# liruiw/OMG-Planner

Hardware: AMD Instinct MI355X
Metric: CHOMP iterations/sec (batched scenes) + ms/plan, Panda 7-DoF 30-wp (higher is better)
Workload: dtype f32 SDF / f64 kinematics+update; 1 GPU; 100 table-top scenes/GPU x (64-goal goal-set cost + CHOMP step), Panda 9-dof, 30 waypoints; scenes_per_gpu=100, total_scenes=100, goals=64, waypoints=30, sdf_grid=4x64^3 + 128x96x32 per scene, private, goal_selection=MD on device (omgx_goal_update_optimize), pipeline_parts=3, top_k_collision=1000, plan_restart_every_steps=50

## Files before the change

### omg-planner_amd/csrc/omg_device.h

```cpp
#pragma once
#include <hip/hip_runtime.h>
#include <stdint.h>

#include "../../include/omg_hip.h"

#define OMG_WAVE 64

namespace omg {

struct __attribute__((packed, aligned(4))) F2 { float a, b; };
struct __attribute__((packed, aligned(4))) F4 { float a, b, c, d; };

__device__ __forceinline__ float lerpf(float a, float b, float t) { return __builtin_fmaf(t, b - a, a); }

struct Axis { int i0; float f; bool ok; };
__device__ __forceinline__ Axis axis_of(float g) {
    Axis a;
    a.ok = (g > -1.0e9f) && (g <= 1.0e9f);
    const float s = g - 0.5f;
    a.i0 = (int)s;
    a.f = s - (float)a.i0;
    const bool edge = (s == -1.0f) && (g > -0.5f);
    a.i0 = edge ? 0 : a.i0;
    a.f = edge ? -1.0f : a.f;
// ... 165 lines not shown
        fmx = sdf_value(G, axm, ay, az);
        fmy = sdf_value(G, ax, aym, az);
        fmz = sdf_value(G, ax, ay, azm);
    }
    const float g0 = (float)(0.5 * (double)(fpx - fmx) * o.rdelta);
    const float g1 = (float)(0.5 * (double)(fpy - fmy) * o.rdelta);
    const float g2 = (float)(0.5 * (double)(fpz - fmz) * o.rdelta);
    float v0, v1, v2;
    if (value <= 0.0f) {
        acc.pot += (float)(-(double)value + 0.5 * (double)o.eps);
        v0 = -g0; v1 = -g1; v2 = -g2;
    } else {
        const float d = value - o.eps;
        acc.pot += o.i2eps * d * d * o.pad;
        const float ie = o.ieps;
        v0 = ie * g0 * d * o.pad; v1 = ie * g1 * d * o.pad; v2 = ie * g2 * d * o.pad;
    }
    acc.gx += __builtin_fmaf(T[8], v2, __builtin_fmaf(T[4], v1, T[0] * v0));
    acc.gy += __builtin_fmaf(T[9], v2, __builtin_fmaf(T[5], v1, T[1] * v0));
    acc.gz += __builtin_fmaf(T[10], v2, __builtin_fmaf(T[6], v1, T[2] * v0));
}

template <bool WANT_GRAD>
__device__ __forceinline__ void sdf_pair(const ObjParams& o, const float* __restrict__ grid, float px, float py, float pz,
                                         Accum& acc) {
    const PairPrep pp = pair_prepare(o, px, py, pz);
    if (!pp.far) pair_exact<WANT_GRAD>(o, grid, pp.tx, pp.ty, pp.tz, acc);
}

#define OMG_CONST_AS __attribute__((address_space(4)))
typedef const OMG_CONST_AS omgx_object* ObjTablePtr;
typedef const OMG_CONST_AS int32_t* IntTablePtr;
#define OMG_GLOBAL_AS __attribute__((address_space(1)))
typedef const OMG_GLOBAL_AS char* GlobalBytes;
typedef float F2v __attribute__((ext_vector_type(2), aligned(4)));
__device__ __forceinline__ F2 global_f2(GlobalBytes p) { const F2v v = *(const OMG_GLOBAL_AS F2v*)p; return F2{v.x, v.y}; }
__device__ __forceinline__ ObjTablePtr as_const(const omgx_object* p) { return (ObjTablePtr)(uintptr_t)p; }
__device__ __forceinline__ IntTablePtr as_const(const int32_t* p) { return (IntTablePtr)(uintptr_t)p; }

__device__ __forceinline__ ObjParams load_object(ObjTablePtr ob) {
    ObjParams o;
#pragma unroll
    for (int k = 0; k < 12; ++k) o.T[k] = ob->pose_inv[k];
#pragma unroll
    for (int k = 0; k < 3; ++k) { o.lo[k] = ob->lo[k]; o.hi[k] = ob->hi[k]; o.dim[k] = ob->dim[k]; }
    o.delta = ob->delta; o.eps = ob->epsilon; o.pad = ob->padding_scale; o.clr = ob->clearance;
#pragma unroll
    for (int k = 0; k < 3; ++k) { o.rw[k] = ob->inv_extent[k]; o.rc[k] = ob->rb_c[k]; o.rh[k] = ob->rb_h[k]; }
    o.rr2 = ob->rb_r2;
    o.rdelta = ob->inv_delta; o.i2eps = ob->inv_2eps; o.ieps = ob->inv_eps;
    return o;
}

template <bool WANT_GRAD>
__device__ __forceinline__ Accum sdf_point(const omgx_object* __restrict__ objs, int o_begin, int o_end,
                                           const float* __restrict__ pool, float px, float py, float pz) {
    Accum acc{0.0f, 0.0f, 0.0f, 0.0f, 0.0f};
    for (int o = o_begin; o < o_end; ++o) {
        ObjTablePtr ob = as_const(objs) + o;
        if (ob->disabled > 0) continue;
        const ObjParams op = load_object(ob);
        sdf_pair<WANT_GRAD>(op, pool + ob->grid_offset, px, py, pz, acc);
    }
    return acc;
}

__device__ __forceinline__ void gq_warm_scalar_cache(const omgx_object* objects, int o_begin, int o_end, const double* balls) {
    const omgx_object* ob[8];
#pragma unroll
    for (int k = 0; k < 8; ++k) ob[k] = objects + (o_begin + k < o_end ? o_begin + k : o_end - 1);
#define OMG_WARM_OBJ(N) "s_load_dword s96, %" #N ", 0x0\n\ts_load_dword s97, %" #N ", 0x40\n\ts_load_dword s98, %" #N ", 0x80\n\ts_load_dword s99, %" #N ", 0xb4\n\t"
    asm volatile(OMG_WARM_OBJ(0) OMG_WARM_OBJ(1) OMG_WARM_OBJ(2) OMG_WARM_OBJ(3) OMG_WARM_OBJ(4) OMG_WARM_OBJ(5) OMG_WARM_OBJ(6) OMG_WARM_OBJ(7)
                 "s_load_dword s96, %8, 0x0\n\ts_load_dword s97, %8, 0x40\n\ts_load_dword s98, %8, 0x80\n\ts_load_dword s99, %8, 0xc0\n\t"
                 "s_load_dword s96, %8, 0x100\n\ts_load_dword s97, %8, 0x13c\n\ts_waitcnt lgkmcnt(0)"
                 :
                 : "s"(ob[0]), "s"(ob[1]), "s"(ob[2]), "s"(ob[3]), "s"(ob[4]), "s"(ob[5]), "s"(ob[6]), "s"(ob[7]), "s"(balls)
                 : "s96", "s97", "s98", "s99", "memory");
#undef OMG_WARM_OBJ
}

template <class DPtr>
struct RobotViewT {
    const double* __restrict__ raw;
    DPtr d;
    const double* __restrict__ g;
    int P;
    __device__ __forceinline__ RobotViewT(const double* blob, int P_) : raw(blob), d((DPtr)(uintptr_t)(blob + OMGX_ROBOT_POINTS + 30 * P_)), g(blob + OMGX_ROBOT_POINTS + 30 * P_), P(P_) {}
    __device__ __forceinline__ RobotViewT(const double* blob, int P_, DPtr chain_constants) : raw(blob), d(chain_constants), g(blob + OMGX_ROBOT_POINTS + 30 * P_), P(P_) {}
    __device__ __forceinline__ DPtr uvw(int i) const { return d + 27 * i; }
    __device__ __forceinline__ DPtr tp(int i) const { return d + 189 + 3 * i; }
    __device__ __forceinline__ DPtr hand() const { return d + 210; }
    __device__ __forceinline__ DPtr lf() const { return d + 222; }
    __device__ __forceinline__ DPtr rf() const { return d + 234; }
    __device__ __forceinline__ const double* pts(int l, int p) const { return g + 246 + 3 * (l * P + p); }
    __device__ __forceinline__ DPtr ax(int l) const { return d + 246 + 30 * P + 3 * l; }
    __device__ __forceinline__ DPtr og(int l) const { return d + 276 + 30 * P + 3 * l; }
    __device__ __forceinline__ double radius(int l) const { return d[306 + 30 * P + l]; }
    __device__ __forceinline__ DPtr ball(int l) const { return d + 316 + 30 * P + 4 * l; }
    __device__ __forceinline__ const double* lower() const { return raw + OMGX_ROBOT_LOWER; }
    __device__ __forceinline__ const double* upper() const { return raw + OMGX_ROBOT_UPPER; }
};
typedef RobotViewT<const double*> RobotView;
typedef RobotViewT<const OMG_CONST_AS double*> RobotViewS;

struct Pose { double R[9]; double t[3]; };

// ... 42 lines not shown
            nxt.t[r] = cur.R[3 * r] * tp[0] + cur.R[3 * r + 1] * tp[1] + cur.R[3 * r + 2] * tp[2] + cur.t[r];
        }
        cur = nxt;
        f(i, cur);
    }
    Pose hand;
    pose_mul(cur, rv.hand(), hand);
    f(7, hand);
    {
        double Fm[12];
        const auto L = rv.lf();
#pragma unroll
        for (int k = 0; k < 12; ++k) Fm[k] = L[k];
        Fm[7] += deg_round_trip(q[7]);
        Pose fp;
        pose_mul(hand, Fm, fp);
        f(8, fp);
        const auto Rr = rv.rf();
#pragma unroll
        for (int k = 0; k < 12; ++k) Fm[k] = Rr[k];
        Fm[7] -= deg_round_trip(q[8]);
        pose_mul(hand, Fm, fp);
        f(9, fp);
    }
}

__device__ __forceinline__ void fk_joint_sincos(double q, double& s, double& c) { sincos(deg_round_trip(q), &s, &c); }

__device__ __forceinline__ double fk_dot3(double a0, double a1, double a2, double b0, double b1, double b2) {
#pragma clang fp contract(off)
    return __builtin_fma(a2, b2, __builtin_fma(a1, b1, a0 * b0));
}
__device__ __forceinline__ double fk_bentry(double c, double s, double U, double V, double W) {
#pragma clang fp contract(off)
    return __builtin_fma(s, V, c * U) + W;
}
template <class RV, class F>
__device__ __forceinline__ void fk_chain_tail(const RV& rv, double a0, double a1, double a2, double at, double q7, double q8, F&& f) {
#pragma clang fp contract(off)
    const auto H = rv.hand();
    const double h0 = fk_dot3(a0, a1, a2, H[0], H[4], H[8]), h1 = fk_dot3(a0, a1, a2, H[1], H[5], H[9]), h2 = fk_dot3(a0, a1, a2, H[2], H[6], H[10]);
    const double ht = fk_dot3(a0, a1, a2, H[3], H[7], H[11]) + at;
    f(7, h0, h1, h2, ht);
    const auto Lf = rv.lf();
    f(8, fk_dot3(h0, h1, h2, Lf[0], Lf[4], Lf[8]), fk_dot3(h0, h1, h2, Lf[1], Lf[5], Lf[9]), fk_dot3(h0, h1, h2, Lf[2], Lf[6], Lf[10]),
      fk_dot3(h0, h1, h2, Lf[3], Lf[7] + deg_round_trip(q7), Lf[11]) + ht);
    const auto Rf = rv.rf();
    f(9, fk_dot3(h0, h1, h2, Rf[0], Rf[4], Rf[8]), fk_dot3(h0, h1, h2, Rf[1], Rf[5], Rf[9]), fk_dot3(h0, h1, h2, Rf[2], Rf[6], Rf[10]),
      fk_dot3(h0, h1, h2, Rf[3], Rf[7] - deg_round_trip(q8), Rf[11]) + ht);
}

template <class RV, class F>
__device__ __forceinline__ void fk_chain_row(const RV& rv, int r, const double* __restrict__ sc ,
                                             double q7, double q8, F&& f) {
#pragma clang fp contract(off)
    double a0 = r == 0 ? 1.0 : 0.0, a1 = r == 1 ? 1.0 : 0.0, a2 = r == 2 ? 1.0 : 0.0, at = 0.0;
#pragma unroll 1
    for (int i = 0; i < 7; ++i) {
        const double s = sc[2 * i], c = sc[2 * i + 1];
        const auto uvw = rv.uvw(i);
        const auto tp = rv.tp(i);
        double B[9];
#pragma unroll
        for (int k = 0; k < 9; ++k) B[k] = fk_bentry(c, s, uvw[k], uvw[9 + k], uvw[18 + k]);
        const double n0 = fk_dot3(a0, a1, a2, B[0], B[3], B[6]);
        const double n1 = fk_dot3(a0, a1, a2, B[1], B[4], B[7]);
        const double n2 = fk_dot3(a0, a1, a2, B[2], B[5], B[8]);
        at = fk_dot3(a0, a1, a2, tp[0], tp[1], tp[2]) + at;
        a0 = n0; a1 = n1; a2 = n2;
        f(i, a0, a1, a2, at);
    }
    fk_chain_tail(rv, a0, a1, a2, at, q7, q8, f);
}

template <class RV>
__device__ __forceinline__ void fk_joint_matrix(const RV& rv, int i, double s, double c, double* __restrict__ B) {
    const auto uvw = rv.uvw(i);
#pragma unroll
    for (int k = 0; k < 9; ++k) B[k] = fk_bentry(c, s, uvw[k], uvw[9 + k], uvw[18 + k]);
}

template <class RV, class F>
__device__ __forceinline__ void fk_chain_row_B(const RV& rv, int r, const double* Bt , double q7, double q8, F&& f, int bstride = 9) {
#pragma clang fp contract(off)
    double a0 = r == 0 ? 1.0 : 0.0, a1 = r == 1 ? 1.0 : 0.0, a2 = r == 2 ? 1.0 : 0.0, at = 0.0;
#pragma unroll 1
    for (int i = 0; i < 7; ++i) {
        const double* B = Bt + bstride * i;
        const auto tp = rv.tp(i);
        const double n0 = fk_dot3(a0, a1, a2, B[0], B[3], B[6]);
        const double n1 = fk_dot3(a0, a1, a2, B[1], B[4], B[7]);
        const double n2 = fk_dot3(a0, a1, a2, B[2], B[5], B[8]);
        at = fk_dot3(a0, a1, a2, tp[0], tp[1], tp[2]) + at;
        a0 = n0; a1 = n1; a2 = n2;
        f(i, a0, a1, a2, at);
    }
    fk_chain_tail(rv, a0, a1, a2, at, q7, q8, f);
}

__device__ __forceinline__ void pose_apply(const Pose& A, const double* __restrict__ p, double& x, double& y, double& z) {
#pragma clang fp contract(fast)
    x = A.R[0] * p[0] + A.R[1] * p[1] + A.R[2] * p[2] + A.t[0];
    y = A.R[3] * p[0] + A.R[4] * p[1] + A.R[5] * p[2] + A.t[1];
    z = A.R[6] * p[0] + A.R[7] * p[1] + A.R[8] * p[2] + A.t[2];
}

__device__ __forceinline__ void pose12_apply(const double* __restrict__ A, const double* __restrict__ p, float& x, float& y, float& z) {
#pragma clang fp contract(fast)
    x = (float)(A[0] * p[0] + A[1] * p[1] + A[2] * p[2] + A[9]);
    y = (float)(A[3] * p[0] + A[4] * p[1] + A[5] * p[2] + A[10]);
    z = (float)(A[6] * p[0] + A[7] * p[1] + A[8] * p[2] + A[11]);
}

__device__ __forceinline__ void pose9_apply(const double* __restrict__ A, const double* __restrict__ p, float& x, float& y, float& z) {
#pragma clang fp contract(fast)
    const double r20 = A[1] * A[5] - A[2] * A[4], r21 = A[2] * A[3] - A[0] * A[5], r22 = A[0] * A[4] - A[1] * A[3];
    x = (float)(A[0] * p[0] + A[1] * p[1] + A[2] * p[2] + A[6]);
    y = (float)(A[3] * p[0] + A[4] * p[1] + A[5] * p[2] + A[7]);
    z = (float)(r20 * p[0] + r21 * p[1] + r22 * p[2] + A[8]);
}

template <class BP>
__device__ __forceinline__ void link_ball_center(const double* r0, const double* r1, const double* t, BP b, float& cx, float& cy, float& cz) {
#pragma clang fp contract(off)
    const double c0 = b[0], c1 = b[1], c2 = b[2];
    const double r20 = __builtin_fma(r0[1], r1[2], -(r0[2] * r1[1])), r21 = __builtin_fma(r0[2], r1[0], -(r0[0] * r1[2])),
                 r22 = __builtin_fma(r0[0], r1[1], -(r0[1] * r1[0]));
    cx = (float)(fk_dot3(r0[0], r0[1], r0[2], c0, c1, c2) + t[0]);
    cy = (float)(fk_dot3(r1[0], r1[1], r1[2], c0, c1, c2) + t[1]);
    cz = (float)(fk_dot3(r20, r21, r22, c0, c1, c2) + t[2]);
}

template <bool MIN>
__device__ __forceinline__ bool np_arg_better(double v, int i, double bv, int bi) {
    const bool vn = v != v, bn = bv != bv;
    if (vn | bn) return vn && (!bn || i < bi);
    return (MIN ? v < bv : v > bv) || (v == bv && i < bi);
}

template <int CTRL>
__device__ __forceinline__ int dpp_i32(int v) { return __builtin_amdgcn_update_dpp(0, v, CTRL, 0xf, 0xf, false); }
template <int CTRL>
__device__ __forceinline__ float dpp_f32(float v) { return __int_as_float(dpp_i32<CTRL>(__float_as_int(v))); }
template <int CTRL>
__device__ __forceinline__ double dpp_f64(double v) {
    return __hiloint2double(dpp_i32<CTRL>(__double2hiint(v)), dpp_i32<CTRL>(__double2loint(v)));
}
__device__ __forceinline__ int wave_suffix_sum_i32(int v) {
    v += __builtin_amdgcn_update_dpp(0, v, 0x101, 0xf, 0xf, true);
    v += __builtin_amdgcn_update_dpp(0, v, 0x102, 0xf, 0xf, true);
// ... 37 lines not shown
```

### omg-planner_amd/csrc/omg_goalset_queue.h

```cpp
#pragma once

#define GQ_TBL_MAX 32
#ifndef GQ_WG_PER_CU
#define GQ_WG_PER_CU 5
#endif
#ifndef GQ_WAVES
#define GQ_WAVES 4
#endif
#define GQ_NT (64 * GQ_WAVES)

struct GqFar {
    float T[12], lo[3], rc[3], rh[3], rr2, rb_r;
    bool cullable;
    int disabled;
};

typedef uint32_t GqU16 __attribute__((ext_vector_type(16)));
typedef uint32_t GqU8 __attribute__((ext_vector_type(8)));
typedef uint32_t GqU4 __attribute__((ext_vector_type(4)));
static_assert(offsetof(omgx_object, pose_inv) == 0 && offsetof(omgx_object, lo) == 0x30 && offsetof(omgx_object, epsilon) == 0x58 &&
              offsetof(omgx_object, clearance) == 0x60 && offsetof(omgx_object, disabled) == 0x64 && offsetof(omgx_object, rb_c) == 0x88 &&
              offsetof(omgx_object, rb_h) == 0x94 && offsetof(omgx_object, rb_r) == 0xa0 && offsetof(omgx_object, rb_r2) == 0xa4 &&
              sizeof(omgx_object) >= 0xa8, "gq_load_far reads the record by byte offsets");
__device__ __forceinline__ GqFar gq_load_far(ObjTablePtr ob) {
    GqU16 a;
    GqU4 b;
    GqU8 c;
    asm volatile("s_load_dwordx16 %0, %3, 0x0\n\ts_load_dwordx4 %1, %3, 0x58\n\ts_load_dwordx8 %2, %3, 0x88\n\ts_waitcnt lgkmcnt(0)"
                 : "=&s"(a), "=&s"(b), "=&s"(c) : "s"((uint64_t)(uintptr_t)ob));
    GqFar f;
#pragma unroll
    for (int k = 0; k < 12; ++k) f.T[k] = __uint_as_float(a[k]);
#pragma unroll
    for (int k = 0; k < 3; ++k) { f.lo[k] = __uint_as_float(a[12 + k]); f.rc[k] = __uint_as_float(c[k]); f.rh[k] = __uint_as_float(c[3 + k]); }
    f.rb_r = __uint_as_float(c[6]);
    f.rr2 = __uint_as_float(c[7]);
    f.cullable = ((int32_t)b[0] < 0x3f800000) & ((int32_t)b[2] <= 0x3f800000);
    f.disabled = (int32_t)b[3];
    return f;
}
__device__ __forceinline__ void se3_apply_s(const float* T, float x, float y, float z, float& ux, float& uy, float& uz) {
    ux = T[3]; uy = T[7]; uz = T[11];
    asm("v_fma_f32 %0, %3, %12, %0\n\tv_fma_f32 %1, %6, %12, %1\n\tv_fma_f32 %2, %9, %12, %2\n\t"
        "v_fma_f32 %0, %4, %13, %0\n\tv_fma_f32 %1, %7, %13, %1\n\tv_fma_f32 %2, %10, %13, %2\n\t"
        "v_fma_f32 %0, %5, %14, %0\n\tv_fma_f32 %1, %8, %14, %1\n\tv_fma_f32 %2, %11, %14, %2"
        : "+v"(ux), "+v"(uy), "+v"(uz)
        : "s"(T[0]), "s"(T[1]), "s"(T[2]), "s"(T[4]), "s"(T[5]), "s"(T[6]), "s"(T[8]), "s"(T[9]), "s"(T[10]), "v"(x), "v"(y), "v"(z));
}
__device__ __forceinline__ unsigned long long wave_ballot(bool b) { return __builtin_amdgcn_ballot_w64(b); }

struct GqLayout {
    int mask_off, tile_off, tbl_off, pts_off, stage_off, fkc_off, objc_off, btab_off, total;
    __host__ __device__ GqLayout(int PS, int MR, int P, int tbl_n, bool with_fkc = false, int waves = GQ_WAVES) {
        mask_off = PS * 90 * 8;
        tile_off = mask_off + 10 * MR * 4;
        tbl_off = mask_off + ((10 * MR * 4 + 16 + 15) & ~15);
        pts_off = tbl_off + tbl_n * 64;
        stage_off = pts_off + ((10 * P * 3 * 8 + 15) & ~15);
        total = stage_off + waves * 64 * 16;
        const int fk = stage_off + PS * 14 * 8 + 16;
        if (total < fk) total = fk;
        total = (total + 15) & ~15;
        fkc_off = total;
        if (with_fkc) total += 246 * 8;
        objc_off = total;
        if (with_fkc) total += 8 * 64 * 5 * 4;
        btab_off = total;
        if (with_fkc) total += PS * 7 * 9 * 8;
    }
};

static inline int gq_choose_tbl_n(int PS, int MR, int P, bool with_fkc = false, int waves = GQ_WAVES) {
    static const int step[] = {26624, 31744, 40960, 53248, 80896, 163840};
    const int base = GqLayout(PS, MR, P, 0, with_fkc, waves).total;
    for (int k = 0; k < 6; ++k)
        if (base + 4 * 64 <= step[k]) {
            const int n = (step[k] - base) / 64;
            return n < GQ_TBL_MAX ? n : GQ_TBL_MAX;
        }
    return 0;
}

struct GqTblRec { double rw[3]; int32_t dim[3]; int64_t goffb; float eps, clr, pad, i2e; };
__device__ __forceinline__ GqTblRec gq_tbl_load(const omgx_object* ob) {
    GqTblRec r;
#pragma unroll
    for (int k = 0; k < 3; ++k) { r.rw[k] = ob->inv_extent[k]; r.dim[k] = ob->dim[k]; }
    r.goffb = ob->grid_offset * 4;
    r.eps = ob->epsilon; r.clr = ob->clearance; r.pad = ob->padding_scale; r.i2e = ob->inv_2eps;
    return r;
}
__device__ __forceinline__ void gq_tbl_store(uint32_t* e, const GqTblRec& r) {
#pragma unroll
// ... 690 lines not shown
```

### omg-planner_amd/csrc/omg_kernels.hip

```cpp
#include <hip/hip_runtime.h>
#include <hip/hip_ext.h>

#include <stdint.h>
#include <stdio.h>
#include <stdlib.h>
#include <string.h>

#include <mutex>

#include "omg_device.h"
#include "omg_host.h"

using namespace omg;

struct RawObjects {
    const float* __restrict__ pose_init;
    const float* __restrict__ sdf_grids;
    const float* __restrict__ sdf_limits;
    const float* __restrict__ eps;
    const float* __restrict__ pad;
    const float* __restrict__ clr;
    const float* __restrict__ dis;
};

// ... 239 lines not shown
                        if (!__any((many & bit) != 0)) continue;
                        ObjTablePtr ob = as_const(a.objects) + o;
                        if (ob->disabled > 0) continue;
                        const ObjParams op = load_object(ob);
                        const float* grid = a.pool + ob->grid_offset;
                        PairPrep pp[LB];
#pragma unroll
                        for (int k = 0; k < LB; ++k) {
                            pp[k] = pair_prepare(op, px[k], py[k], pz[k]);
                            pp[k].far = pp[k].far || !(msk[k] & bit);
                        }
#pragma unroll
                        for (int k = 0; k < LB; ++k)
                            if (!pp[k].far) pair_exact<WANT_GRAD>(op, grid, pp[k].tx, pp[k].ty, pp[k].tz, acc[k]);
                    }
                }
#pragma unroll
                for (int k = 0; k < LB; ++k) {
                    const int l = l0 + k;
                    if (a.soften && l >= 8) {
                        acc[k].pot *= 0.1f; acc[k].gx *= 0.1f; acc[k].gy *= 0.1f; acc[k].gz *= 0.1f; acc[k].col = 0.0f;
                    }
                    if (a.arc && acc[k].pot != 0.0f) {
                        float qx, qy, qz;
                        pose12_apply(ci > 0 ? base + ((int64_t)l * pstride + ci - 1) * 12 : sbase + (int64_t)l * sstride, rv.pts(l, p), qx, qy, qz);
                        const float vx = (px[k] - qx) * a.inv_dt, vy = (py[k] - qy) * a.inv_dt, vz = (pz[k] - qz) * a.inv_dt;
                        acc[k].pot = acc[k].pot * sqrtf(vx * vx + vy * vy + vz * vz);
                    }
                    const int64_t kk = (out_cfg + l) * P + p;
                    if (a.pot) a.pot[kk] = acc[k].pot;
                    if (a.col) a.col[kk] = acc[k].col;
                    if (WANT_GRAD) { a.grad[3 * kk] = acc[k].gx; a.grad[3 * kk + 1] = acc[k].gy; a.grad[3 * kk + 2] = acc[k].gz; }
                    tsum += acc[k].pot;
                    tcol += acc[k].col;
                }
            }
        }
    }
    if (a.chunk_cost || a.chunk_col) {
        const float ws_ = wave_sum(tsum), wc_ = wave_sum(tcol);
        const int w = threadIdx.x >> 6;
        if ((threadIdx.x & 63) == 0) { red[0][w] = ws_; red[1][w] = wc_; }
        __syncthreads();
        if (threadIdx.x == 0) {
            const int64_t k = (int64_t)s * a.NCH + chunk;
            float c0 = red[0][0], c1 = red[1][0];
#pragma unroll
            for (int w2 = 1; w2 < TPB / 64; ++w2) { c0 += red[0][w2]; c1 += red[1][w2]; }
            if (a.chunk_cost) a.chunk_cost[k] = c0;
            if (a.chunk_col) a.chunk_col[k] = c1;
        }
    }
}
template <bool LAT, bool PERSIST = false>
__device__ __forceinline__ void waypoint_layer_block(const ChunkArgs& a, const int s, const int l_begin, const int l_end,
                                                     const int c_begin, const int c_end, double* lds_pose, uint32_t* rowmask,
                                                     const int o_begin, const int o_end, const RobotViewS& rv, double* fkc,
                                                     const bool warming, float* objc, double* btab) {
    const int n = a.wp_n, P = a.P, PS = a.PS, MR = a.MR;
    const int nloc = c_end - c_begin;
    const double* tr = a.wp_traj + ((int64_t)s * n + c_begin) * 9;
    double* sc = reinterpret_cast<double*>(rowmask);
    auto ldtr = [&](int k) -> double {
        if constexpr (PERSIST) return __hip_atomic_load(tr + k, __ATOMIC_RELAXED, __HIP_MEMORY_SCOPE_AGENT);
        else return tr[k];
    };
    const double fkv = (LAT && threadIdx.x < 246) ? rv.g[threadIdx.x] : 0.0;
    if (warming) gq_warm_scalar_cache(a.objects, o_begin, o_end, a.robot + OMGX_ROBOT_POINTS + 30 * P + 316 + 30 * P);
    for (int t = threadIdx.x; t < nloc * 7; t += 256) {
        const int cfg = t / 7, i = t - cfg * 7;
        double sn, cs;
        fk_joint_sincos(ldtr(cfg * 9 + i), sn, cs);
        sc[2 * t] = sn; sc[2 * t + 1] = cs;
    }
    if (LAT && threadIdx.x < 246) fkc[threadIdx.x] = fkv;
    __syncthreads();
    double* const gpose = (a.wp_pose_out && l_begin == 0) ? a.wp_pose_out + ((int64_t)s * n + c_begin) * 120 : nullptr;
    auto run_chain = [&](const auto& view) {
        for (int t = threadIdx.x; t < nloc * 3; t += 256) {
            const int cfg = t / 3, r = t - cfg * 3;
            fk_chain_row(view, r, sc + 14 * cfg, ldtr(cfg * 9 + 7), ldtr(cfg * 9 + 8), [&](int l, double r0, double r1, double r2, double tt) {
                double* dst = lds_pose + ((size_t)l * PS + cfg) * 9;
                if (r < 2) { dst[3 * r] = r0; dst[3 * r + 1] = r1; dst[3 * r + 2] = r2; }
                dst[6 + r] = tt;
                if (gpose) {
                    double* g = gpose + ((size_t)cfg * 10 + l) * 12;
                    g[3 * r] = r0; g[3 * r + 1] = r1; g[3 * r + 2] = r2; g[9 + r] = tt;
                }
            });
        }
    };
    if constexpr (LAT) {
        const RobotView rvl(a.robot, P, fkc);
        for (int t = threadIdx.x; t < nloc * 7; t += 256) fk_joint_matrix(rvl, t - (t / 7) * 7, sc[2 * t], sc[2 * t + 1], btab + 9 * t);
        __syncthreads();
        for (int t = threadIdx.x; t < nloc * 3; t += 256) {
            const int cfg = t / 3, r = t - cfg * 3;
            fk_chain_row_B(rvl, r, btab + 63 * cfg, ldtr(cfg * 9 + 7), ldtr(cfg * 9 + 8), [&](int l, double r0, double r1, double r2, double tt) {
                double* dst = lds_pose + ((size_t)l * PS + cfg) * 9;
                if (r < 2) { dst[3 * r] = r0; dst[3 * r + 1] = r1; dst[3 * r + 2] = r2; }
                dst[6 + r] = tt;
                if (gpose) {
                    double* g = gpose + ((size_t)cfg * 10 + l) * 12;
                    g[3 * r] = r0; g[3 * r + 1] = r1; g[3 * r + 2] = r2; g[9 + r] = tt;
                }
            });
        }
    } else run_chain(rv);
    __syncthreads();
    for (int row = l_begin * nloc + threadIdx.x; row < l_end * nloc; row += 256) {
        const int l = row / nloc, ci = row - l * nloc;
        const double* A = lds_pose + ((int64_t)l * PS + ci) * 9;
        const auto bl = rv.ball(l);
        float cx, cy, cz;
        link_ball_center(A, A + 3, A + 6, bl, cx, cy, cz);
        const float rad = (float)bl[3] + 1.0e-4f;
        uint32_t m = 0;
        for (int o = o_begin; o < o_end; ++o) {
            ObjTablePtr ob = as_const(a.objects) + o;
            if (ob->disabled > 0) continue;
            const int oo = o - o_begin;
            const uint32_t bit = 1u << (oo < 31 ? oo : 31);
            const float ux = __builtin_fmaf(ob->pose_inv[2], cz, __builtin_fmaf(ob->pose_inv[1], cy, __builtin_fmaf(ob->pose_inv[0], cx, ob->pose_inv[3]))) - ob->lo[0];
            const float uy = __builtin_fmaf(ob->pose_inv[6], cz, __builtin_fmaf(ob->pose_inv[5], cy, __builtin_fmaf(ob->pose_inv[4], cx, ob->pose_inv[7]))) - ob->lo[1];
            const float uz = __builtin_fmaf(ob->pose_inv[10], cz, __builtin_fmaf(ob->pose_inv[9], cy, __builtin_fmaf(ob->pose_inv[8], cx, ob->pose_inv[11]))) - ob->lo[2];
            const float rbc[3] = {ob->rb_c[0], ob->rb_c[1], ob->rb_c[2]}, rbh[3] = {ob->rb_h[0], ob->rb_h[1], ob->rb_h[2]};
            const bool near = rbox_near(ux, uy, uz, rad, rbc, rbh, ob->rb_r);
            const bool cullable = ob->epsilon < 1.0f && ob->clearance <= 1.0f;
            if (near || !cullable) m |= bit;
        }
        rowmask[l * MR + ci] = m;
    }
    __syncthreads();
    if (LAT && nloc <= 4 && l_end - l_begin == 1) {
        const int l = l_begin, lane = threadIdx.x & 63, wave = threadIdx.x >> 6;
        const int p = lane & 15, ci = lane >> 4;
        const bool valid = (p < P) && (ci < nloc);
        const int cic = valid ? ci : 0, pc = valid ? p : 0;
        const uint32_t msk = valid ? rowmask[l * MR + cic] : 0u;
        Accum acc{0.0f, 0.0f, 0.0f, 0.0f, 0.0f};
        if (__any(msk != 0)) {
            float px, py, pz;
            pose9_apply(lds_pose + ((int64_t)l * PS + cic) * 9, rv.pts(l, pc), px, py, pz);
            for (int og = o_begin; og < o_end; og += 8) {
                for (int o = og + wave; o < og + 8 && o < o_end; o += 4) {
                    const int oo = o - o_begin;
                    const uint32_t bit = 1u << (oo < 31 ? oo : 31);
                    Accum c{0.0f, 0.0f, 0.0f, 0.0f, 0.0f};
                    if (__any((msk & bit) != 0)) {
                        ObjTablePtr ob = as_const(a.objects) + o;
                        if (!(ob->disabled > 0)) {
                            const ObjParams op = load_object(ob);
                            const PairPrep pp = pair_prepare(op, px, py, pz);
                            if ((msk & bit) && !pp.far) pair_exact<true>(op, a.pool + ob->grid_offset, pp.tx, pp.ty, pp.tz, c);
                        }
                    }
                    float* dst = objc + ((o - og) * 64 + lane) * 5;
                    dst[0] = c.pot; dst[1] = c.gx; dst[2] = c.gy; dst[3] = c.gz; dst[4] = c.col;
                }
                __syncthreads();
                if (wave == 0) {
                    for (int o = og; o < og + 8 && o < o_end; ++o) {
                        const float* src = objc + ((o - og) * 64 + lane) * 5;
                        acc.pot += src[0]; acc.gx += src[1]; acc.gy += src[2]; acc.gz += src[3]; acc.col += src[4];
                    }
                }
                __syncthreads();
            }
        }
        if (wave == 0) {
            if (a.wp_soften && l >= 8) {
                acc.pot *= 0.1f; acc.gx *= 0.1f; acc.gy *= 0.1f; acc.gz *= 0.1f; acc.col = 0.0f;
            }
            if (valid) {
                const int64_t kk = (((int64_t)s * n + c_begin + ci) * 10 + l) * P + p;
                a.wp_pot[kk] = acc.pot;
                a.wp_col[kk] = acc.col;
                a.wp_grad[3 * kk] = acc.gx; a.wp_grad[3 * kk + 1] = acc.gy; a.wp_grad[3 * kk + 2] = acc.gz;
            }
        }
        return;
    }
    const int p = threadIdx.x & 15, r = threadIdx.x >> 4;
    for (int ci0 = 0; ci0 < nloc; ci0 += 16) {
        const int ci = ci0 + r;
        const bool valid = (p < P) && (ci < nloc);
        const int cic = valid ? ci : 0, pc = valid ? p : 0;
#pragma unroll 1
        for (int l = l_begin; l < l_end; ++l) {
            const uint32_t msk = valid ? rowmask[l * MR + cic] : 0u;
            Accum acc{0.0f, 0.0f, 0.0f, 0.0f, 0.0f};
            if (__any(msk != 0)) {
                float px, py, pz;
                pose9_apply(lds_pose + ((int64_t)l * PS + cic) * 9, rv.pts(l, pc), px, py, pz);
                for (int o = o_begin; o < o_end; ++o) {
                    const int oo = o - o_begin;
                    const uint32_t bit = 1u << (oo < 31 ? oo : 31);
                    if (!__any((msk & bit) != 0)) continue;
                    ObjTablePtr ob = as_const(a.objects) + o;
                    if (ob->disabled > 0) continue;
                    const ObjParams op = load_object(ob);
                    const PairPrep pp = pair_prepare(op, px, py, pz);
                    if ((msk & bit) && !pp.far) pair_exact<true>(op, a.pool + ob->grid_offset, pp.tx, pp.ty, pp.tz, acc);
                }
            }
            if (a.wp_soften && l >= 8) {
                acc.pot *= 0.1f; acc.gx *= 0.1f; acc.gy *= 0.1f; acc.gz *= 0.1f; acc.col = 0.0f;
            }
            if (valid) {
                const int64_t kk = (((int64_t)s * n + c_begin + ci) * 10 + l) * P + p;
                a.wp_pot[kk] = acc.pot;
                a.wp_col[kk] = acc.col;
                a.wp_grad[3 * kk] = acc.gx; a.wp_grad[3 * kk + 1] = acc.gy; a.wp_grad[3 * kk + 2] = acc.gz;
            }
        }
    }
}

#ifdef OMGX_GS_CLOCK
__device__ unsigned long long g_gs_wg[1 << 16][8];
#define GS_WG_IDX ((blockIdx.x + (((unsigned)a.S & 1u) << 14)) & 0xffffu)
#define GS_WG_STAMP(k) do { if (threadIdx.x == 0 && blockIdx.x < (1u << 16)) { g_gs_wg[GS_WG_IDX][k] = wall_clock64(); if (k == 0) { g_gs_wg[GS_WG_IDX][5] = ~0ull; g_gs_wg[GS_WG_IDX][6] = 0ull; unsigned hw, xcc; asm volatile("s_getreg_b32 %0, hwreg(HW_REG_HW_ID)" : "=s"(hw)); asm volatile("s_getreg_b32 %0, hwreg(HW_REG_XCC_ID)" : "=s"(xcc)); g_gs_wg[GS_WG_IDX][7] = ((unsigned long long)xcc << 32) | hw; } } } while (0)
__device__ unsigned long long g_gs_wave[1 << 16][8];
#define GS_WAVE_STAMP(k) do { if ((threadIdx.x & 63) == 0 && (k) < 8 && blockIdx.x < (1u << 16)) g_gs_wave[blockIdx.x][k] = wall_clock64(); } while (0)
extern "C" int omgx_debug_gs_wave(unsigned long long* h_out, int n_wg) {
    if (n_wg > (1 << 16)) n_wg = 1 << 16;
    return hipMemcpyFromSymbol(h_out, HIP_SYMBOL(g_gs_wave), sizeof(unsigned long long) * 8 * n_wg) == hipSuccess ? 0 : -2;
}
__device__ unsigned long long g_gs_freq[1 << 16][2];
#define GS_FREQ_BEGIN() unsigned long long gs_f0 = 0, gs_f1 = 0; if (threadIdx.x == 0) { gs_f0 = __builtin_readcyclecounter(); gs_f1 = wall_clock64(); }
#define GS_FREQ_END() do { if (threadIdx.x == 0 && blockIdx.x < (1u << 16)) { g_gs_freq[blockIdx.x][0] = __builtin_readcyclecounter() - gs_f0; g_gs_freq[blockIdx.x][1] = wall_clock64() - gs_f1; } } while (0)
extern "C" int omgx_debug_gs_freq(unsigned long long* h_out, int n_wg) {
    if (n_wg > (1 << 16)) n_wg = 1 << 16;
    return hipMemcpyFromSymbol(h_out, HIP_SYMBOL(g_gs_freq), sizeof(unsigned long long) * 2 * n_wg) == hipSuccess ? 0 : -2;
}
extern "C" int omgx_debug_gs_wg(unsigned long long* h_out, int n_wg) {
    if (n_wg > (1 << 16)) n_wg = 1 << 16;
    return hipMemcpyFromSymbol(h_out, HIP_SYMBOL(g_gs_wg), sizeof(unsigned long long) * 8 * n_wg) == hipSuccess ? 0 : -2;
}
#else
#define GS_WG_STAMP(k)
#define GS_WAVE_STAMP(k)
#define GS_FREQ_BEGIN()
#define GS_FREQ_END()
#endif

#if defined(OMGX_GS_ADD_S)
#define GS_MARGINAL_COST_PROBE(a_, b_, c_, d_, i_, j_) do { { uint32_t d0 = (uint32_t)(i_), d1 = (uint32_t)(j_); asm volatile("s_add_u32 %0, %0, 3\n\ts_add_u32 %1, %1, 5\n\ts_add_u32 %0, %0, 3\n\ts_add_u32 %1, %1, 5\n\ts_add_u32 %0, %0, 3\n\ts_add_u32 %1, %1, 5\n\ts_add_u32 %0, %0, 3\n\ts_add_u32 %1, %1, 5\n\t" "s_add_u32 %0, %0, 3\n\ts_add_u32 %1, %1, 5\n\ts_add_u32 %0, %0, 3\n\ts_add_u32 %1, %1, 5\n\ts_add_u32 %0, %0, 3\n\ts_add_u32 %1, %1, 5\n\ts_add_u32 %0, %0, 3\n\ts_add_u32 %1, %1, 5" : "+s"(d0), "+s"(d1) : : "scc"); } } while (0)
#elif defined(OMGX_GS_ADD_V)
#define GS_MARGINAL_COST_PROBE(a_, b_, c_, d_, i_, j_) do { { float d0 = (a_), d1 = (b_), d2 = (c_), d3 = (d_); asm volatile("v_fma_f32 %0, %0, %0, %0\n\tv_fma_f32 %1, %1, %1, %1\n\tv_fma_f32 %2, %2, %2, %2\n\tv_fma_f32 %3, %3, %3, %3\n\t" "v_fma_f32 %0, %0, %0, %0\n\tv_fma_f32 %1, %1, %1, %1\n\tv_fma_f32 %2, %2, %2, %2\n\tv_fma_f32 %3, %3, %3, %3\n\t" "v_fma_f32 %0, %0, %0, %0\n\tv_fma_f32 %1, %1, %1, %1\n\tv_fma_f32 %2, %2, %2, %2\n\tv_fma_f32 %3, %3, %3, %3\n\t" "v_fma_f32 %0, %0, %0, %0\n\tv_fma_f32 %1, %1, %1, %1\n\tv_fma_f32 %2, %2, %2, %2\n\tv_fma_f32 %3, %3, %3, %3" : "+v"(d0), "+v"(d1), "+v"(d2), "+v"(d3)); } } while (0)
#elif defined(OMGX_GS_ADD_V64)
#define GS_MARGINAL_COST_PROBE(a_, b_, c_, d_, i_, j_) do { { double d0 = (a_), d1 = (b_), d2 = (c_), d3 = (d_); asm volatile("v_fma_f64 %0, %0, %0, %0\n\tv_fma_f64 %1, %1, %1, %1\n\tv_fma_f64 %2, %2, %2, %2\n\tv_fma_f64 %3, %3, %3, %3\n\t" "v_fma_f64 %0, %0, %0, %0\n\tv_fma_f64 %1, %1, %1, %1\n\tv_fma_f64 %2, %2, %2, %2\n\tv_fma_f64 %3, %3, %3, %3\n\t" "v_fma_f64 %0, %0, %0, %0\n\tv_fma_f64 %1, %1, %1, %1\n\tv_fma_f64 %2, %2, %2, %2\n\tv_fma_f64 %3, %3, %3, %3\n\t" "v_fma_f64 %0, %0, %0, %0\n\tv_fma_f64 %1, %1, %1, %1\n\tv_fma_f64 %2, %2, %2, %2\n\tv_fma_f64 %3, %3, %3, %3" : "+v"(d0), "+v"(d1), "+v"(d2), "+v"(d3)); } } while (0)
#elif defined(OMGX_GS_ADD_B)
#define GS_MARGINAL_COST_PROBE(a_, b_, c_, d_, i_, j_) do { asm volatile("s_branch 1f\n\ts_nop 0\n\t1:\n\ts_branch 2f\n\ts_nop 0\n\t2:\n\ts_branch 3f\n\ts_nop 0\n\t3:\n\ts_branch 4f\n\ts_nop 0\n\t4:\n\t" "s_branch 5f\n\ts_nop 0\n\t5:\n\ts_branch 6f\n\ts_nop 0\n\t6:\n\ts_branch 7f\n\ts_nop 0\n\t7:\n\ts_branch 8f\n\ts_nop 0\n\t8:"); } while (0)
#elif defined(OMGX_GS_ADD_N)
#define GS_MARGINAL_COST_PROBE(a_, b_, c_, d_, i_, j_) do { asm volatile("s_nop 0\n\ts_nop 0\n\ts_nop 0\n\ts_nop 0\n\ts_nop 0\n\ts_nop 0\n\ts_nop 0\n\ts_nop 0\n\ts_nop 0\n\ts_nop 0\n\ts_nop 0\n\ts_nop 0\n\ts_nop 0\n\ts_nop 0\n\ts_nop 0\n\ts_nop 0"); } while (0)
// ... 899 lines not shown
```

Measured before the change: 564,600 iterations/s.

## Truncate FK chain to needed layers and batch scalar object-record loads

The waypoint layer block now stops the forward-kinematics chain at the last link layer it needs. Sincos and joint matrices for unused joints are skipped, and the pose-output condition is adjusted to match. Object records are fetched as a few wide scalar loads (gq_load_far moved to the common header, plus a new load_object_whole), replacing many separate field loads. Per-wave vote checks are replaced by readlane ORs of the row masks. The hand-written byte-offset asm is tied to the struct layout, and skipping FK work changes which poses get written.

```diff
diff --git a/omg-planner_amd/csrc/omg_device.h b/omg-planner_amd/csrc/omg_device.h
--- a/omg-planner_amd/csrc/omg_device.h
+++ b/omg-planner_amd/csrc/omg_device.h
@@ -241,6 +241,77 @@
     return o;
 }
 
+struct GqFar {
+    float T[12], lo[3], rc[3], rh[3], rr2, rb_r;
+    float eps, clr;
+    bool cullable;
+    int disabled;
+};
+
+typedef uint32_t GqU16 __attribute__((ext_vector_type(16)));
+typedef uint32_t GqU8 __attribute__((ext_vector_type(8)));
+typedef uint32_t GqU4 __attribute__((ext_vector_type(4)));
+typedef uint32_t GqU2 __attribute__((ext_vector_type(2)));
+static_assert(offsetof(omgx_object, pose_inv) == 0 && offsetof(omgx_object, lo) == 0x30 && offsetof(omgx_object, epsilon) == 0x58 &&
+              offsetof(omgx_object, clearance) == 0x60 && offsetof(omgx_object, disabled) == 0x64 && offsetof(omgx_object, rb_c) == 0x88 &&
+              offsetof(omgx_object, rb_h) == 0x94 && offsetof(omgx_object, rb_r) == 0xa0 && offsetof(omgx_object, rb_r2) == 0xa4 &&
+              sizeof(omgx_object) >= 0xa8, "gq_load_far reads the record by byte offsets");
+__device__ __forceinline__ GqFar gq_load_far(ObjTablePtr ob) {
+    GqU16 a;
+    GqU4 b;
+    GqU8 c;
+    asm volatile("s_load_dwordx16 %0, %3, 0x0\n\ts_load_dwordx4 %1, %3, 0x58\n\ts_load_dwordx8 %2, %3, 0x88\n\ts_waitcnt lgkmcnt(0)"
+                 : "=&s"(a), "=&s"(b), "=&s"(c) : "s"((uint64_t)(uintptr_t)ob));
+    GqFar f;
+#pragma unroll
+    for (int k = 0; k < 12; ++k) f.T[k] = __uint_as_float(a[k]);
+#pragma unroll
+    for (int k = 0; k < 3; ++k) { f.lo[k] = __uint_as_float(a[12 + k]); f.rc[k] = __uint_as_float(c[k]); f.rh[k] = __uint_as_float(c[3 + k]); }
+    f.rb_r = __uint_as_float(c[6]);
+    f.rr2 = __uint_as_float(c[7]);
+    f.eps = __uint_as_float(b[0]); f.clr = __uint_as_float(b[2]);
+    f.cullable = ((int32_t)b[0] < 0x3f800000) & ((int32_t)b[2] <= 0x3f800000);
+    f.disabled = (int32_t)b[3];
+    return f;
+}
+
+struct ObjWhole { ObjParams op; int disabled; int64_t grid_offset; };
+static_assert(offsetof(omgx_object, hi) == 0x3c && offsetof(omgx_object, dim) == 0x48 && offsetof(omgx_object, delta) == 0x54 &&
+              offsetof(omgx_object, padding_scale) == 0x5c && offsetof(omgx_object, grid_offset) == 0x68 &&
+              offsetof(omgx_object, inv_extent) == 0x70 && offsetof(omgx_object, inv_delta) == 0xa8 && offsetof(omgx_object, inv_2eps) == 0xb0 &&
+              offsetof(omgx_object, inv_eps) == 0xb4 && sizeof(omgx_object) == 0xb8, "load_object_whole reads the record by byte offsets");
+__device__ __forceinline__ ObjWhole load_object_whole(ObjTablePtr ob) {
+    GqU16 a, b;
+    GqU8 c;
+    GqU4 d;
+    GqU2 e;
+    asm volatile("s_load_dwordx16 %0, %5, 0x0\n\ts_load_dwordx16 %1, %5, 0x40\n\ts_load_dwordx8 %2, %5, 0x80\n\t"
+                 "s_load_dwordx4 %3, %5, 0xa0\n\ts_load_dwordx2 %4, %5, 0xb0\n\ts_waitcnt lgkmcnt(0)"
+                 : "=&s"(a), "=&s"(b), "=&s"(c), "=&s"(d), "=&s"(e) : "s"((uint64_t)(uintptr_t)ob));
+    ObjWhole w;
+    ObjParams& o = w.op;
+#pragma unroll
+    for (int k = 0; k < 12; ++k) o.T[k] = __uint_as_float(a[k]);
+#pragma unroll
+    for (int k = 0; k < 3; ++k) {
+        o.lo[k] = __uint_as_float(a[12 + k]);
+        o.dim[k] = (int)b[2 + k];
+        o.rc[k] = __uint_as_float(c[2 + k]);
+        o.rh[k] = __uint_as_float(c[5 + k]);
+    }
+    o.hi[0] = __uint_as_float(a[15]); o.hi[1] = __uint_as_float(b[0]); o.hi[2] = __uint_as_float(b[1]);
+    o.delta = __uint_as_float(b[5]); o.eps = __uint_as_float(b[6]); o.pad = __uint_as_float(b[7]); o.clr = __uint_as_float(b[8]);
+    w.disabled = (int32_t)b[9];
+    w.grid_offset = (int64_t)(((uint64_t)b[11] << 32) | (uint64_t)b[10]);
+    o.rw[0] = __hiloint2double((int)b[13], (int)b[12]);
+    o.rw[1] = __hiloint2double((int)b[15], (int)b[14]);
+    o.rw[2] = __hiloint2double((int)c[1], (int)c[0]);
+    o.rr2 = __uint_as_float(d[1]);
+    o.rdelta = __hiloint2double((int)d[3], (int)d[2]);
+    o.i2eps = __uint_as_float(e[0]); o.ieps = __uint_as_float(e[1]);
+    return w;
+}
+
 template <bool WANT_GRAD>
 __device__ __forceinline__ Accum sdf_point(const omgx_object* __restrict__ objs, int o_begin, int o_end,
                                            const float* __restrict__ pool, float px, float py, float pz) {
@@ -389,11 +460,12 @@
 
 template <class RV, class F>
 __device__ __forceinline__ void fk_chain_row(const RV& rv, int r, const double* __restrict__ sc ,
-                                             double q7, double q8, F&& f) {
+                                             double q7, double q8, F&& f, const int l_stop = 10 ) {
 #pragma clang fp contract(off)
     double a0 = r == 0 ? 1.0 : 0.0, a1 = r == 1 ? 1.0 : 0.0, a2 = r == 2 ? 1.0 : 0.0, at = 0.0;
+    const int nj = l_stop < 7 ? l_stop : 7;
 #pragma unroll 1
-    for (int i = 0; i < 7; ++i) {
+    for (int i = 0; i < nj; ++i) {
         const double s = sc[2 * i], c = sc[2 * i + 1];
         const auto uvw = rv.uvw(i);
         const auto tp = rv.tp(i);
@@ -407,7 +479,7 @@
         a0 = n0; a1 = n1; a2 = n2;
         f(i, a0, a1, a2, at);
     }
-    fk_chain_tail(rv, a0, a1, a2, at, q7, q8, f);
+    if (l_stop > 7) fk_chain_tail(rv, a0, a1, a2, at, q7, q8, f);
 }
 
 template <class RV>
@@ -418,11 +490,13 @@
 }
 
 template <class RV, class F>
-__device__ __forceinline__ void fk_chain_row_B(const RV& rv, int r, const double* Bt , double q7, double q8, F&& f, int bstride = 9) {
+__device__ __forceinline__ void fk_chain_row_B(const RV& rv, int r, const double* Bt , double q7, double q8, F&& f, int bstride = 9,
+                                               const int l_stop = 10) {
 #pragma clang fp contract(off)
     double a0 = r == 0 ? 1.0 : 0.0, a1 = r == 1 ? 1.0 : 0.0, a2 = r == 2 ? 1.0 : 0.0, at = 0.0;
+    const int nj = l_stop < 7 ? l_stop : 7;
 #pragma unroll 1
-    for (int i = 0; i < 7; ++i) {
+    for (int i = 0; i < nj; ++i) {
         const double* B = Bt + bstride * i;
         const auto tp = rv.tp(i);
         const double n0 = fk_dot3(a0, a1, a2, B[0], B[3], B[6]);
@@ -432,7 +506,7 @@
         a0 = n0; a1 = n1; a2 = n2;
         f(i, a0, a1, a2, at);
     }
-    fk_chain_tail(rv, a0, a1, a2, at, q7, q8, f);
+    if (l_stop > 7) fk_chain_tail(rv, a0, a1, a2, at, q7, q8, f);
 }
 
 __device__ __forceinline__ void pose_apply(const Pose& A, const double* __restrict__ p, double& x, double& y, double& z) {
diff --git a/omg-planner_amd/csrc/omg_goalset_queue.h b/omg-planner_amd/csrc/omg_goalset_queue.h
--- a/omg-planner_amd/csrc/omg_goalset_queue.h
+++ b/omg-planner_amd/csrc/omg_goalset_queue.h
@@ -9,36 +9,6 @@
 #endif
 #define GQ_NT (64 * GQ_WAVES)
 
-struct GqFar {
-    float T[12], lo[3], rc[3], rh[3], rr2, rb_r;
-    bool cullable;
-    int disabled;
-};
-
-typedef uint32_t GqU16 __attribute__((ext_vector_type(16)));
-typedef uint32_t GqU8 __attribute__((ext_vector_type(8)));
-typedef uint32_t GqU4 __attribute__((ext_vector_type(4)));
-static_assert(offsetof(omgx_object, pose_inv) == 0 && offsetof(omgx_object, lo) == 0x30 && offsetof(omgx_object, epsilon) == 0x58 &&
-              offsetof(omgx_object, clearance) == 0x60 && offsetof(omgx_object, disabled) == 0x64 && offsetof(omgx_object, rb_c) == 0x88 &&
-              offsetof(omgx_object, rb_h) == 0x94 && offsetof(omgx_object, rb_r) == 0xa0 && offsetof(omgx_object, rb_r2) == 0xa4 &&
-              sizeof(omgx_object) >= 0xa8, "gq_load_far reads the record by byte offsets");
-__device__ __forceinline__ GqFar gq_load_far(ObjTablePtr ob) {
-    GqU16 a;
-    GqU4 b;
-    GqU8 c;
-    asm volatile("s_load_dwordx16 %0, %3, 0x0\n\ts_load_dwordx4 %1, %3, 0x58\n\ts_load_dwordx8 %2, %3, 0x88\n\ts_waitcnt lgkmcnt(0)"
-                 : "=&s"(a), "=&s"(b), "=&s"(c) : "s"((uint64_t)(uintptr_t)ob));
-    GqFar f;
-#pragma unroll
-    for (int k = 0; k < 12; ++k) f.T[k] = __uint_as_float(a[k]);
-#pragma unroll
-    for (int k = 0; k < 3; ++k) { f.lo[k] = __uint_as_float(a[12 + k]); f.rc[k] = __uint_as_float(c[k]); f.rh[k] = __uint_as_float(c[3 + k]); }
-    f.rb_r = __uint_as_float(c[6]);
-    f.rr2 = __uint_as_float(c[7]);
-    f.cullable = ((int32_t)b[0] < 0x3f800000) & ((int32_t)b[2] <= 0x3f800000);
-    f.disabled = (int32_t)b[3];
-    return f;
-}
 __device__ __forceinline__ void se3_apply_s(const float* T, float x, float y, float z, float& ux, float& uy, float& uz) {
     ux = T[3]; uy = T[7]; uz = T[11];
     asm("v_fma_f32 %0, %3, %12, %0\n\tv_fma_f32 %1, %6, %12, %1\n\tv_fma_f32 %2, %9, %12, %2\n\t"
diff --git a/omg-planner_amd/csrc/omg_kernels.hip b/omg-planner_amd/csrc/omg_kernels.hip
--- a/omg-planner_amd/csrc/omg_kernels.hip
+++ b/omg-planner_amd/csrc/omg_kernels.hip
@@ -315,6 +315,10 @@
         }
     }
 }
+__device__ __forceinline__ uint32_t wave_rows_mask(uint32_t msk) {
+    return (uint32_t)(__builtin_amdgcn_readlane((int)msk, 0) | __builtin_amdgcn_readlane((int)msk, 16) |
+                      __builtin_amdgcn_readlane((int)msk, 32) | __builtin_amdgcn_readlane((int)msk, 48));
+}
 template <bool LAT, bool PERSIST = false>
 __device__ __forceinline__ void waypoint_layer_block(const ChunkArgs& a, const int s, const int l_begin, const int l_end,
                                                      const int c_begin, const int c_end, double* lds_pose, uint32_t* rowmask,
@@ -330,15 +334,18 @@
     };
     const double fkv = (LAT && threadIdx.x < 246) ? rv.g[threadIdx.x] : 0.0;
     if (warming) gq_warm_scalar_cache(a.objects, o_begin, o_end, a.robot + OMGX_ROBOT_POINTS + 30 * P + 316 + 30 * P);
+    const int l_stop = LAT ? 10 : l_end;
+    const int nj = l_stop < 7 ? l_stop : 7;
     for (int t = threadIdx.x; t < nloc * 7; t += 256) {
         const int cfg = t / 7, i = t - cfg * 7;
+        if (i >= nj) continue;
         double sn, cs;
         fk_joint_sincos(ldtr(cfg * 9 + i), sn, cs);
         sc[2 * t] = sn; sc[2 * t + 1] = cs;
     }
     if (LAT && threadIdx.x < 246) fkc[threadIdx.x] = fkv;
     __syncthreads();
-    double* const gpose = (a.wp_pose_out && l_begin == 0) ? a.wp_pose_out + ((int64_t)s * n + c_begin) * 120 : nullptr;
+    double* const gpose = (a.wp_pose_out && l_end == 10) ? a.wp_pose_out + ((int64_t)s * n + c_begin) * 120 : nullptr;
     auto run_chain = [&](const auto& view) {
         for (int t = threadIdx.x; t < nloc * 3; t += 256) {
             const int cfg = t / 3, r = t - cfg * 3;
@@ -350,12 +357,13 @@
                     double* g = gpose + ((size_t)cfg * 10 + l) * 12;
                     g[3 * r] = r0; g[3 * r + 1] = r1; g[3 * r + 2] = r2; g[9 + r] = tt;
                 }
-            });
+            }, l_stop);
         }
     };
     if constexpr (LAT) {
         const RobotView rvl(a.robot, P, fkc);
-        for (int t = threadIdx.x; t < nloc * 7; t += 256) fk_joint_matrix(rvl, t - (t / 7) * 7, sc[2 * t], sc[2 * t + 1], btab + 9 * t);
+        for (int t = threadIdx.x; t < nloc * 7; t += 256)
+            if (t - (t / 7) * 7 < nj) fk_joint_matrix(rvl, t - (t / 7) * 7, sc[2 * t], sc[2 * t + 1], btab + 9 * t);
         __syncthreads();
         for (int t = threadIdx.x; t < nloc * 3; t += 256) {
             const int cfg = t / 3, r = t - cfg * 3;
@@ -367,7 +375,7 @@
                     double* g = gpose + ((size_t)cfg * 10 + l) * 12;
                     g[3 * r] = r0; g[3 * r + 1] = r1; g[3 * r + 2] = r2; g[9 + r] = tt;
                 }
-            });
+            }, 9, l_stop);
         }
     } else run_chain(rv);
     __syncthreads();
@@ -380,29 +388,30 @@
         const float rad = (float)bl[3] + 1.0e-4f;
         uint32_t m = 0;
         for (int o = o_begin; o < o_end; ++o) {
-            ObjTablePtr ob = as_const(a.objects) + o;
-            if (ob->disabled > 0) continue;
+            const GqFar f = gq_load_far(as_const(a.objects) + o);
+            if (f.disabled > 0) continue;
             const int oo = o - o_begin;
             const uint32_t bit = 1u << (oo < 31 ? oo : 31);
-            const float ux = __builtin_fmaf(ob->pose_inv[2], cz, __builtin_fmaf(ob->pose_inv[1], cy, __builtin_fmaf(ob->pose_inv[0], cx, ob->pose_inv[3]))) - ob->lo[0];
-            const float uy = __builtin_fmaf(ob->pose_inv[6], cz, __builtin_fmaf(ob->pose_inv[5], cy, __builtin_fmaf(ob->pose_inv[4], cx, ob->pose_inv[7]))) - ob->lo[1];
-            const float uz = __builtin_fmaf(ob->pose_inv[10], cz, __builtin_fmaf(ob->pose_inv[9], cy, __builtin_fmaf(ob->pose_inv[8], cx, ob->pose_inv[11]))) - ob->lo[2];
-            const float rbc[3] = {ob->rb_c[0], ob->rb_c[1], ob->rb_c[2]}, rbh[3] = {ob->rb_h[0], ob->rb_h[1], ob->rb_h[2]};
-            const bool near = rbox_near(ux, uy, uz, rad, rbc, rbh, ob->rb_r);
-            const bool cullable = ob->epsilon < 1.0f && ob->clearance <= 1.0f;
+            const float ux = __builtin_fmaf(f.T[2], cz, __builtin_fmaf(f.T[1], cy, __builtin_fmaf(f.T[0], cx, f.T[3]))) - f.lo[0];
+            const float uy = __builtin_fmaf(f.T[6], cz, __builtin_fmaf(f.T[5], cy, __builtin_fmaf(f.T[4], cx, f.T[7]))) - f.lo[1];
+            const float uz = __builtin_fmaf(f.T[10], cz, __builtin_fmaf(f.T[9], cy, __builtin_fmaf(f.T[8], cx, f.T[11]))) - f.lo[2];
+            const bool near = rbox_near(ux, uy, uz, rad, f.rc, f.rh, f.rb_r);
+            const bool cullable = f.eps < 1.0f && f.clr <= 1.0f;
             if (near || !cullable) m |= bit;
         }
         rowmask[l * MR + ci] = m;
     }
     __syncthreads();
     if (LAT && nloc <= 4 && l_end - l_begin == 1) {
-        const int l = l_begin, lane = threadIdx.x & 63, wave = threadIdx.x >> 6;
+        const int l = l_begin, lane = threadIdx.x & 63;
+        const int wave = __builtin_amdgcn_readfirstlane((int)(threadIdx.x >> 6));
         const int p = lane & 15, ci = lane >> 4;
         const bool valid = (p < P) && (ci < nloc);
         const int cic = valid ? ci : 0, pc = valid ? p : 0;
         const uint32_t msk = valid ? rowmask[l * MR + cic] : 0u;
         Accum acc{0.0f, 0.0f, 0.0f, 0.0f, 0.0f};
-        if (__any(msk != 0)) {
+        const uint32_t sm = wave_rows_mask(msk);
+        if (sm != 0) {
             float px, py, pz;
             pose9_apply(lds_pose + ((int64_t)l * PS + cic) * 9, rv.pts(l, pc), px, py, pz);
             for (int og = o_begin; og < o_end; og += 8) {
@@ -410,12 +419,11 @@
                     const int oo = o - o_begin;
                     const uint32_t bit = 1u << (oo < 31 ? oo : 31);
                     Accum c{0.0f, 0.0f, 0.0f, 0.0f, 0.0f};
-                    if (__any((msk & bit) != 0)) {
-                        ObjTablePtr ob = as_const(a.objects) + o;
-                        if (!(ob->disabled > 0)) {
-                            const ObjParams op = load_object(ob);
-                            const PairPrep pp = pair_prepare(op, px, py, pz);
-                            if ((msk & bit) && !pp.far) pair_exact<true>(op, a.pool + ob->grid_offset, pp.tx, pp.ty, pp.tz, c);
+                    if (sm & bit) {
+                        const ObjWhole ow = load_object_whole(as_const(a.objects) + o);
+                        if (!(ow.disabled > 0)) {
+                            const PairPrep pp = pair_prepare(ow.op, px, py, pz);
+                            if ((msk & bit) && !pp.far) pair_exact<true>(ow.op, a.pool + ow.grid_offset, pp.tx, pp.ty, pp.tz, c);
                         }
                     }
                     float* dst = objc + ((o - og) * 64 + lane) * 5;
@@ -453,18 +461,18 @@
         for (int l = l_begin; l < l_end; ++l) {
             const uint32_t msk = valid ? rowmask[l * MR + cic] : 0u;
             Accum acc{0.0f, 0.0f, 0.0f, 0.0f, 0.0f};
-            if (__any(msk != 0)) {
+            const uint32_t sm = wave_rows_mask(msk);
+            if (sm != 0) {
                 float px, py, pz;
                 pose9_apply(lds_pose + ((int64_t)l * PS + cic) * 9, rv.pts(l, pc), px, py, pz);
                 for (int o = o_begin; o < o_end; ++o) {
                     const int oo = o - o_begin;
                     const uint32_t bit = 1u << (oo < 31 ? oo : 31);
-                    if (!__any((msk & bit) != 0)) continue;
-                    ObjTablePtr ob = as_const(a.objects) + o;
-                    if (ob->disabled > 0) continue;
-                    const ObjParams op = load_object(ob);
-                    const PairPrep pp = pair_prepare(op, px, py, pz);
-                    if ((msk & bit) && !pp.far) pair_exact<true>(op, a.pool + ob->grid_offset, pp.tx, pp.ty, pp.tz, acc);
+                    if (!(sm & bit)) continue;
+                    const ObjWhole ow = load_object_whole(as_const(a.objects) + o);
+                    if (ow.disabled > 0) continue;
+                    const PairPrep pp = pair_prepare(ow.op, px, py, pz);
+                    if ((msk & bit) && !pp.far) pair_exact<true>(ow.op, a.pool + ow.grid_offset, pp.tx, pp.ty, pp.tz, acc);
                 }
             }
             if (a.wp_soften && l >= 8) {
```

Result: no change. 563,600 iterations/s (-0.2%).
